# xswang/xflow

Measured on NVIDIA H100. Metric: training examples/sec, higher is better.
Workload: dtype f32

## Files before the change

### xflow_b200/csrc/step_lazy.cu

```cuda
#include <cuda_runtime.h>
#include <stdint.h>
#include <stdlib.h>

#include "kernels.h"
#include "table.cuh"

#define XF_NO_SLOT 0xFFFFFFFFu
#define XF_LAZY_CACHED 2

__global__ void __launch_bounds__(256, 3)
xf_k_step_lr_lazy(XfTableView t, const uint32_t* __restrict__ row_ptr, const uint64_t* __restrict__ keys,
                  const uint8_t* __restrict__ labels, int B, int mode, uint32_t seq, uint32_t* rows_by_seq,
                  float* __restrict__ loss_out, float* __restrict__ pctr_out, float* __restrict__ abs_loss_sum,
                  unsigned long long* __restrict__ unique_total) {
  __shared__ float s_abs[8];
  __shared__ unsigned int s_open;
  if (threadIdx.x == 0) s_open = 0;
  if (blockIdx.x == 0 && threadIdx.x == 0 && mode == 0) rows_by_seq[seq] = (uint32_t)B;
  __syncthreads();
  float abs_acc = 0.f;
  unsigned int open_acc = 0;
  const int lane = threadIdx.x & 31;
  const int warps_per_block = blockDim.x >> 5;
  const int gwarp = blockIdx.x * warps_per_block + (threadIdx.x >> 5);
  const int nwarps = gridDim.x * warps_per_block;

  for (int row = gwarp; row < B; row += nwarps) {
    const uint32_t beg = __ldg(row_ptr + row);
    const uint32_t end = __ldg(row_ptr + row + 1);
    const int chunks = (int)((end - beg + 63u) >> 6);
    float wsum = 0.f;
    uint32_t lead_s[2 * XF_LAZY_CACHED];
    uint32_t cnt_c[XF_LAZY_CACHED];
    uint64_t q2_c[2 * XF_LAZY_CACHED], q3_c[2 * XF_LAZY_CACHED], q2n_c[2 * XF_LAZY_CACHED];
#pragma unroll
    for (int c = 0; c < XF_LAZY_CACHED; ++c) {
      lead_s[2 * c] = lead_s[2 * c + 1] = XF_NO_SLOT;
      q2_c[2 * c] = q2_c[2 * c + 1] = q3_c[2 * c] = q3_c[2 * c + 1] = q2n_c[2 * c] = q2n_c[2 * c + 1] = 0ull;
      cnt_c[c] = 0;
    }

    for (int ch = 0; ch < chunks; ++ch) {
      const uint32_t j0 = beg + (uint32_t)ch * 64u + (uint32_t)lane;
      const uint32_t j1 = j0 + 32u;
      const bool v0 = j0 < end, v1 = j1 < end;
      const uint64_t k0 = v0 ? __ldcs(keys + j0) : 0ull;
      const uint64_t k1 = v1 ? __ldcs(keys + j1) : 0ull;
      const uint64_t p0 = xf_home_slot(t, k0), p1 = xf_home_slot(t, k1);
      XfHead h0, h1;
      h0.key = h1.key = XF_EMPTY_KEY;
      h0.flags = h1.flags = 0u;
      h0.w = h0.n = h0.z = h1.w = h1.n = h1.z = 0.f;
      h0.g = h1.g = 0.0;
      if (v0) h0 = xf_load_head(xf_row(t, p0));
      if (v1) h1 = xf_load_head(xf_row(t, p1));
      uint32_t s0 = XF_NO_SLOT, s1 = XF_NO_SLOT;
      if (v0) { const int64_t r = xf_probe_from<true>(t, k0, p0, h0); if (r >= 0) s0 = (uint32_t)r; }
      if (v1) { const int64_t r = xf_probe_from<true>(t, k1, p1, h1); if (r >= 0) s1 = (uint32_t)r; }
      const uint64_t a2 = xf_raw_q2(h0), a3 = xf_raw_q3(h0), b2 = xf_raw_q2(h1), b3 = xf_raw_q3(h1);
      uint64_t a2n = a2, b2n = b2;
      float w0 = 0.f, w1 = 0.f;
      if (s0 != XF_NO_SLOT) w0 = xf_lazy_fold(t, xf_raw_q1(h0), a2, a3, mode == 1 ? 0xFFFFFFFFu : seq, a2n);
      if (s1 != XF_NO_SLOT) w1 = xf_lazy_fold(t, xf_raw_q1(h1), b2, b3, mode == 1 ? 0xFFFFFFFFu : seq, b2n);
      wsum += w0;
      wsum += w1;
      if (mode == 1) continue;
      const unsigned grp0 = __match_any_sync(0xffffffffu, (s0 != XF_NO_SLOT) ? s0 : (0xFFFFFF00u | (uint32_t)lane));
      const unsigned grp1 = __match_any_sync(0xffffffffu, (s1 != XF_NO_SLOT) ? s1 : (0xFFFFFF00u | (uint32_t)lane));
      const bool L0 = s0 != XF_NO_SLOT && lane == __ffs(grp0) - 1, L1 = s1 != XF_NO_SLOT && lane == __ffs(grp1) - 1;
      if (ch >= XF_LAZY_CACHED) {
        if (L0 && xf_lazy_deposit(t, xf_row(t, s0), a2, a3, a2n, seq, 0ll)) ++open_acc;
        if (L1 && xf_lazy_deposit(t, xf_row(t, s1), b2, b3, b2n, seq, 0ll)) ++open_acc;
      }
#pragma unroll
      for (int c = 0; c < XF_LAZY_CACHED; ++c)
        if (ch == c) {
          lead_s[2 * c] = L0 ? s0 : XF_NO_SLOT;
          lead_s[2 * c + 1] = L1 ? s1 : XF_NO_SLOT;
          q2_c[2 * c] = a2; q3_c[2 * c] = a3; q2n_c[2 * c] = a2n;
          q2_c[2 * c + 1] = b2; q3_c[2 * c + 1] = b3; q2n_c[2 * c + 1] = b2n;
          cnt_c[c] = (L0 ? (uint32_t)__popc(grp0) : 0u) | ((L1 ? (uint32_t)__popc(grp1) : 0u) << 8);
        }
    }

    const float wx = xf_warp_sum(wsum);
    const float pctr = xf_sigmoid(wx);
    if (mode == 1) {
      if (lane == 0 && pctr_out) pctr_out[row] = pctr;
      continue;
    }
    const float loss = __fsub_rn(pctr, (float)labels[row]);
    if (lane == 0 && loss_out) loss_out[row] = loss;
    abs_acc += fabsf(loss);
    const long long lf = xf_fix_of(loss);
#pragma unroll
    for (int c = 0; c < XF_LAZY_CACHED; ++c) {
      if (lead_s[2 * c] != XF_NO_SLOT &&
          xf_lazy_deposit(t, xf_row(t, lead_s[2 * c]), q2_c[2 * c], q3_c[2 * c], q2n_c[2 * c], seq, lf * (long long)(cnt_c[c] & 0xFFu)))
        ++open_acc;
      if (lead_s[2 * c + 1] != XF_NO_SLOT &&
          xf_lazy_deposit(t, xf_row(t, lead_s[2 * c + 1]), q2_c[2 * c + 1], q3_c[2 * c + 1], q2n_c[2 * c + 1], seq,
                          lf * (long long)(cnt_c[c] >> 8)))
        ++open_acc;
    }
    for (int ch = XF_LAZY_CACHED; ch < chunks; ++ch) {
      const uint32_t j0 = beg + (uint32_t)ch * 64u + (uint32_t)lane;
      const uint32_t j1 = j0 + 32u;
      XfHead h;
      if (j0 < end) { const int64_t r = xf_probe<false>(t, __ldg(keys + j0), &h); if (r >= 0) xf_lazy_add(xf_row(t, (uint64_t)r), lf); }
      if (j1 < end) { const int64_t r = xf_probe<false>(t, __ldg(keys + j1), &h); if (r >= 0) xf_lazy_add(xf_row(t, (uint64_t)r), lf); }
    }
  }
  if (mode == 0) {
    if (lane == 0) s_abs[threadIdx.x >> 5] = abs_acc;
    if (open_acc) atomicAdd(&s_open, open_acc);
    __syncthreads();
    if (threadIdx.x == 0) {
      if (abs_loss_sum != nullptr) {
        float tot = 0.f;
        for (int w = 0; w < (int)(blockDim.x >> 5); ++w) tot += s_abs[w];
        atomicAdd(abs_loss_sum, tot);
      }
      if (unique_total != nullptr && s_open) atomicAdd(unique_total, (unsigned long long)s_open);
    }
  }
}

void xf_launch_step_lr_lazy(const XfTableView& t, const uint32_t* row_ptr, const uint64_t* keys,
                            const uint8_t* labels, int B, int mode, uint32_t seq, uint32_t* rows_by_seq,
                            float* loss_out, float* pctr_out, float* abs_loss_sum, unsigned long long* unique_total,
                            cudaStream_t st) {
  if (B <= 0) return;
  const int grid = xf_grid_for((uint64_t)B * 32, 256, 8);
  xf_k_step_lr_lazy<<<grid, 256, 0, st>>>(t, row_ptr, keys, labels, B, mode, seq, rows_by_seq, loss_out, pctr_out,
                                           abs_loss_sum, unique_total);
}
```

### xflow_b200/csrc/table.cuh

```cuda
#pragma once
#include <cuda_runtime.h>
#include <stdint.h>

#define XF_EMPTY_KEY 0xFFFFFFFFFFFFFFFFull
#define XF_FLAG_V_READY 1u
#define XF_NEG_ZERO_BITS 0x80000000u
#define XF_NEG_ZERO_BITS64 0x8000000000000000ull
#define XF_MAX_PROBE 8192

enum { XF_OPT_FTRL = 0, XF_OPT_SGD = 1 };
enum { XF_INIT_DEFAULT = 0, XF_INIT_COUNTER = 1, XF_INIT_ZERO = 3 };

struct XfTableView {
  uint8_t* base;
  uint64_t mask;
  uint32_t log2cap;
  uint32_t bshift;
  uint32_t stride;
  int K;
  int opt;
  int v_init;
  float v_const;
  uint64_t seed;
  float alpha, beta, lambda1, lambda2, learning_rate;
  unsigned long long* size;
  int* error;
  int lazy;
  const uint32_t* rows_by_seq;
  int canon;
};
#define XF_TAG_LOCKED 0xFFFFFFFFu
#define XF_FIX_SCALE 134217728.0
#define XF_FIX_INV 7.450580596923828125e-9
#define XF_TAG_MASK 0xFFFFull

__host__ __device__ inline uint32_t xf_acc_off(int K) { return (32u + 4u * (uint32_t)K + 15u) & ~15u; }
__host__ __device__ inline uint32_t xf_ca_off(int K, int opt) {
  return xf_acc_off(K) + 16u + ((opt == XF_OPT_FTRL) ? 8u * (uint32_t)K : 0u);
}
__host__ __device__ inline uint32_t xf_row_stride(int K, int opt, int canon = 0) {
  if (K <= 0) return 32u;
  uint32_t bytes = xf_ca_off(K, opt) + (canon ? 4u * (uint32_t)K : 0u);
  return (bytes + 31u) & ~31u;
}

#ifdef __CUDACC__

__device__ __forceinline__ uint64_t xf_probe_slot(const XfTableView& t, uint64_t key, uint32_t i) {
  const uint64_t m = key * 0x9E3779B97F4A7C15ull;
  const uint32_t bs = t.bshift;
  const uint64_t hb = m >> (64 - (t.log2cap - bs));
  const uint32_t b1 = (1u << bs) - 1u;
  const uint32_t j0 = (uint32_t)(m >> 9) & b1;
  const uint32_t k = i >> bs;
  const uint32_t j = (k == 0) ? ((j0 + i) & b1) : (i & b1);
  return (((hb + k) << bs) | j) & t.mask;
}
__device__ __forceinline__ uint64_t xf_home_slot(const XfTableView& t, uint64_t key) { return xf_probe_slot(t, key, 0); }

__host__ __device__ __forceinline__ uint64_t xf_splitmix64(uint64_t x) {
  x += 0x9E3779B97F4A7C15ull;
  x = (x ^ (x >> 30)) * 0xBF58476D1CE4E5B9ull;
  x = (x ^ (x >> 27)) * 0x94D049BB133111EBull;
  return x ^ (x >> 31);
}
__device__ __forceinline__ float xf_counter_normal(uint64_t key, uint32_t k, uint64_t seed) {
  uint64_t base = xf_splitmix64(key ^ xf_splitmix64(seed + 0x632BE59BD9B4E019ull * (uint64_t)(k + 1)));
  uint32_t sum = 0;
#pragma unroll
  for (int r = 0; r < 3; ++r) {
    uint64_t x = xf_splitmix64(base + (uint64_t)r);
    sum += (uint32_t)(x & 0xFFFF) + (uint32_t)((x >> 16) & 0xFFFF) + (uint32_t)((x >> 32) & 0xFFFF) +
           (uint32_t)((x >> 48) & 0xFFFF);
  }
  float u = __fmul_rn((float)((int32_t)sum - 6 * 65535), 1.0f / 65536.0f);
  return __fmul_rn(u, 1e-2f);
}
__device__ __forceinline__ float xf_v_init(const XfTableView& t, uint64_t key, uint32_t k) {
  if (t.v_init == XF_INIT_COUNTER) return xf_counter_normal(key, k, t.seed);
  if (t.v_init == XF_INIT_ZERO) return 0.0f;
  return t.v_const;
}

__device__ __forceinline__ uint8_t* xf_row(const XfTableView& t, uint64_t slot) {
  return t.base + slot * (uint64_t)t.stride;
}
__device__ __forceinline__ double* xf_row_g(uint8_t* row) { return reinterpret_cast<double*>(row + 8); }
#define XF_OFF_STATE 16
#define XF_OFF_FLAGS 28
__device__ __forceinline__ float* xf_row_v(uint8_t* row) { return reinterpret_cast<float*>(row + 32); }
__device__ __forceinline__ double* xf_row_acc(uint8_t* row, int K) { return reinterpret_cast<double*>(row + xf_acc_off(K)); }
__device__ __forceinline__ float* xf_row_nv(uint8_t* row, int K) { return reinterpret_cast<float*>(row + xf_acc_off(K) + 16); }
__device__ __forceinline__ float* xf_row_zv(uint8_t* row, int K) { return xf_row_nv(row, K) + K; }
__device__ __forceinline__ float* xf_row_ca(const XfTableView& t, uint8_t* row) { return reinterpret_cast<float*>(row + xf_ca_off(t.K, t.opt)); }

struct XfHead {
  uint64_t key;
  uint32_t flags;
  float w, n, z;
  double g;
};

__device__ __forceinline__ void xf_ld32_cg(const void* p, uint64_t& q0, uint64_t& q1, uint64_t& q2, uint64_t& q3) {
  asm volatile("ld.global.cg.v2.u64 {%0,%1}, [%4];\n\tld.global.cg.v2.u64 {%2,%3}, [%4+16];"
               : "=l"(q0), "=l"(q1), "=l"(q2), "=l"(q3) : "l"(p));
}
__device__ __forceinline__ void xf_ld32_ca(const void* p, uint64_t& q0, uint64_t& q1, uint64_t& q2, uint64_t& q3) {
  asm volatile("ld.global.ca.v2.u64 {%0,%1}, [%4];\n\tld.global.ca.v2.u64 {%2,%3}, [%4+16];"
               : "=l"(q0), "=l"(q1), "=l"(q2), "=l"(q3) : "l"(p));
}
__device__ __forceinline__ void xf_st32(void* p, uint64_t q0, uint64_t q1, uint64_t q2, uint64_t q3) {
  asm volatile("st.global.v2.u64 [%0], {%1,%2};\n\tst.global.v2.u64 [%0+16], {%3,%4};" ::"l"(p), "l"(q0), "l"(q1),
               "l"(q2), "l"(q3)
               : "memory");
}

__device__ __forceinline__ XfHead xf_load_head(const uint8_t* row) {
  uint64_t q0, q1, q2, q3;
  xf_ld32_cg(row, q0, q1, q2, q3);
  XfHead h;
  h.key = q0;
  h.g = __longlong_as_double((long long)q1);
  h.w = __uint_as_float((uint32_t)q2);
  h.n = __uint_as_float((uint32_t)(q2 >> 32));
  h.z = __uint_as_float((uint32_t)q3);
  h.flags = (uint32_t)(q3 >> 32);
  return h;
}

__device__ __forceinline__ XfHead xf_load_head_l1(const uint8_t* row) {
  uint64_t q0, q1, q2, q3;
  xf_ld32_ca(row, q0, q1, q2, q3);
  XfHead h;
  h.key = q0;
  h.g = __longlong_as_double((long long)q1);
  h.w = __uint_as_float((uint32_t)q2);
  h.n = __uint_as_float((uint32_t)(q2 >> 32));
  h.z = __uint_as_float((uint32_t)q3);
  h.flags = (uint32_t)(q3 >> 32);
  return h;
}

__device__ __forceinline__ void xf_ld8_l1(const float* p, float (&o)[8]) {
  uint64_t q0, q1, q2, q3;
  xf_ld32_ca(p, q0, q1, q2, q3);
  o[0] = __uint_as_float((uint32_t)q0); o[1] = __uint_as_float((uint32_t)(q0 >> 32));
  o[2] = __uint_as_float((uint32_t)q1); o[3] = __uint_as_float((uint32_t)(q1 >> 32));
  o[4] = __uint_as_float((uint32_t)q2); o[5] = __uint_as_float((uint32_t)(q2 >> 32));
  o[6] = __uint_as_float((uint32_t)q3); o[7] = __uint_as_float((uint32_t)(q3 >> 32));
}

__device__ __forceinline__ void xf_store_head(uint8_t* row, const XfHead& h) {
  const uint64_t q1 = (uint64_t)__double_as_longlong(h.g);
  const uint64_t q2 = (uint64_t)__float_as_uint(h.w) | ((uint64_t)__float_as_uint(h.n) << 32);
  const uint64_t q3 = (uint64_t)__float_as_uint(h.z) | ((uint64_t)h.flags << 32);
  xf_st32(row, h.key, q1, q2, q3);
}

template <bool INSERT>
__device__ __forceinline__ int64_t xf_probe_from(const XfTableView& t, uint64_t key, uint64_t s, XfHead& h) {
  for (int probes = 0; probes < XF_MAX_PROBE; ++probes) {
    if (h.key == key) return (int64_t)s;
    if (h.key == XF_EMPTY_KEY) {
      if (!INSERT) return -1;
      unsigned long long old =
          atomicCAS(reinterpret_cast<unsigned long long*>(xf_row(t, s)), (unsigned long long)XF_EMPTY_KEY,
                    (unsigned long long)key);
      if (old == XF_EMPTY_KEY) {
        unsigned m = __activemask();
        int leader = __ffs(m) - 1;
        if ((int)(threadIdx.x & 31) == leader) atomicAdd(t.size, (unsigned long long)__popc(m));
        h.key = key; h.flags = 0; h.w = 0.f; h.n = 0.f; h.z = 0.f;
        h.g = t.lazy ? 0.0 : -0.0;
        return (int64_t)s;
      }
      if (old == key) {
        h.key = key;
        return (int64_t)s;
      }
    }
    s = xf_probe_slot(t, key, (uint32_t)probes + 1u);
    h = xf_load_head(xf_row(t, s));
  }
  *t.error = 1;
  return -1;
}

template <bool INSERT>
__device__ __forceinline__ int64_t xf_probe(const XfTableView& t, uint64_t key, XfHead* head) {
  const uint64_t s = xf_home_slot(t, key);
  XfHead h = xf_load_head(xf_row(t, s));
  const int64_t r = xf_probe_from<INSERT>(t, key, s, h);
  *head = h;
  return r;
}


__device__ __forceinline__ float xf_sigmoid(float x) {
  if (x < -30.f) return (float)1e-6;
  if (x > 30.f) return 1.0f;
  const double ex = exp((double)x * 0.9999999998311266);
  return (float)(ex / (1.0 + ex));
}

__device__ __forceinline__ void xf_ftrl_coord(const XfTableView& t, float g, float& w, float& n, float& z) {
  float old_n = n;
  float nn = __fadd_rn(old_n, __fmul_rn(g, g));
  float sig = __fdiv_rn(__fsub_rn(__fsqrt_rn(nn), __fsqrt_rn(old_n)), t.alpha);
  z = __fadd_rn(z, __fsub_rn(g, __fmul_rn(sig, w)));
  n = nn;
  if (fabsf(z) <= t.lambda1) {
    w = 0.0f;
  } else {
    float tmpr = 0.0f;
    if (z > 0.0f) tmpr = __fsub_rn(z, t.lambda1);
    if (z < 0.0f) tmpr = __fadd_rn(z, t.lambda1);
    float tmpl = -__fadd_rn(__fdiv_rn(__fadd_rn(t.beta, __fsqrt_rn(n)), t.alpha), t.lambda2);
    w = __fdiv_rn(tmpr, tmpl);
  }
}

__device__ __forceinline__ void xf_sgd_coord(const XfTableView& t, float g, float& w) {
  w = __fsub_rn(w, __fmul_rn(t.learning_rate, g));
}

__device__ __forceinline__ void xf_opt_coord(const XfTableView& t, float g, float& w, float& n, float& z) {
  if (t.opt == XF_OPT_FTRL) xf_ftrl_coord(t, g, w, n, z);
  else xf_sgd_coord(t, g, w);
}

__device__ __forceinline__ float xf_div_rows_plain(float g, double rows) { return (float)((double)g / rows); }
__device__ __forceinline__ float xf_div_rows(float g, double rows) {
  const long long b = __double_as_longlong(rows);
  if ((b & 0x000FFFFFFFFFFFFFll) == 0ll && b > 0ll) {
    const double inv = __longlong_as_double((2046ll << 52) - b);
    return (float)((double)g * inv);
  }
  return (float)((double)g / rows);
}

__device__ __forceinline__ float xf_ftrl_w(const XfTableView& t, float z, float n) {
  if (fabsf(z) <= t.lambda1) return 0.0f;
  float tmpr = 0.0f;
  if (z > 0.0f) tmpr = __fsub_rn(z, t.lambda1);
  if (z < 0.0f) tmpr = __fadd_rn(z, t.lambda1);
  const float tmpl = -__fadd_rn(__fdiv_rn(__fadd_rn(t.beta, __fsqrt_rn(n)), t.alpha), t.lambda2);
  return __fdiv_rn(tmpr, tmpl);
}
__device__ __forceinline__ long long xf_fix_of(float residual) { return __double2ll_rn((double)residual * XF_FIX_SCALE); }

__device__ __forceinline__ uint64_t xf_raw_q2(const XfHead& h) {
  return (uint64_t)__float_as_uint(h.w) | ((uint64_t)__float_as_uint(h.n) << 32);
}
__device__ __forceinline__ uint64_t xf_raw_q3(const XfHead& h) {
  return (uint64_t)__float_as_uint(h.z) | ((uint64_t)h.flags << 32);
}
__device__ __forceinline__ uint64_t xf_raw_q1(const XfHead& h) { return (uint64_t)__double_as_longlong(h.g); }
__device__ __forceinline__ uint32_t xf_lazy_check(uint64_t q2) {
  const uint32_t c = (uint32_t)q2 ^ (uint32_t)(q2 >> 32) ^ 0xA5A5A5A5u;
  return c ? c : 1u;
}
__device__ __forceinline__ float xf_lazy_fold(const XfTableView& t, uint64_t q1, uint64_t q2, uint64_t q3, uint32_t seq,
                                              uint64_t& q2_new) {
  const uint32_t tag = (uint32_t)(q3 & XF_TAG_MASK);
  const bool pending = tag != 0u && tag != seq;
  float g = 0.f;
  if (pending) {
    const long long gfix = (long long)q3 >> 16;
    g = xf_div_rows_plain((float)((double)gfix * XF_FIX_INV), (double)__ldg(t.rows_by_seq + tag));
  }
  const float a = __uint_as_float((uint32_t)q2), b = __uint_as_float((uint32_t)(q2 >> 32));
  if (t.opt == XF_OPT_FTRL) {
    float n = a, z = b;
    float w = ((uint32_t)(q1 >> 32) == xf_lazy_check(q2)) ? __uint_as_float((uint32_t)q1) : xf_ftrl_w(t, z, n);
    if (pending) xf_ftrl_coord(t, g, w, n, z);
    q2_new = (uint64_t)__float_as_uint(n) | ((uint64_t)__float_as_uint(z) << 32);
    return w;
  }
  float w = a;
  if (pending) xf_sgd_coord(t, g, w);
  q2_new = (uint64_t)__float_as_uint(w);
  return w;
}
__device__ __forceinline__ void xf_apply_pending(const XfTableView& t, XfHead& h) {
  if (!t.lazy) return;
  uint64_t q2n;
  const float w = xf_lazy_fold(t, xf_raw_q1(h), xf_raw_q2(h), xf_raw_q3(h), 0xFFFFFFFFu, q2n);
  h.w = w;
  if (t.opt == XF_OPT_FTRL) {
    h.n = __uint_as_float((uint32_t)q2n);
    h.z = __uint_as_float((uint32_t)(q2n >> 32));
  } else {
    h.n = 0.f;
    h.z = 0.f;
  }
  h.flags = 0u;
  h.g = 0.0;
}
__device__ __forceinline__ bool xf_lazy_has_pending(const XfHead& raw) { return (xf_raw_q3(raw) & XF_TAG_MASK) != 0ull; }
__device__ __forceinline__ void xf_lazy_store(const XfTableView& t, uint8_t* rowp, const XfHead& h, bool keep_w = false) {
  const bool ftrl = t.opt == XF_OPT_FTRL;
  const uint64_t q2 = ftrl ? ((uint64_t)__float_as_uint(h.n) | ((uint64_t)__float_as_uint(h.z) << 32))
                           : (uint64_t)__float_as_uint(h.w);
  uint64_t q1 = 0ull;
  if (keep_w && ftrl && __float_as_uint(h.w) != __float_as_uint(xf_ftrl_w(t, h.z, h.n)))
    q1 = (uint64_t)__float_as_uint(h.w) | ((uint64_t)xf_lazy_check(q2) << 32);
  xf_st32(rowp, h.key, q1, q2, 0ull);
}
__device__ __forceinline__ void xf_store_head_t(const XfTableView& t, uint8_t* rowp, const XfHead& h) {
  if (t.lazy) xf_lazy_store(t, rowp, h);
  else xf_store_head(rowp, h);
}

__device__ __forceinline__ bool xf_cas128(uint8_t* addr, uint64_t e0, uint64_t e1, uint64_t d0, uint64_t d1, uint64_t& o0,
                                          uint64_t& o1) {
  asm volatile(
      "{\n .reg .b128 cmp, swp, old;\n mov.b128 cmp, {%2, %3};\n mov.b128 swp, {%4, %5};\n"
      " atom.global.cas.b128 old, [%6], cmp, swp;\n mov.b128 {%0, %1}, old;\n}"
      : "=l"(o0), "=l"(o1)
      : "l"(e0), "l"(e1), "l"(d0), "l"(d1), "l"(addr)
      : "memory");
  return o0 == e0 && o1 == e1;
}
__device__ __forceinline__ void xf_lazy_add(uint8_t* rowp, long long fix) {
  atomicAdd(reinterpret_cast<unsigned long long*>(rowp + 24), (unsigned long long)fix << 16);
}
__device__ __forceinline__ bool xf_lazy_deposit_issue(uint8_t* rowp, uint64_t q2, uint64_t q3, uint64_t q2_new, uint32_t seq,
                                                      long long fix, uint64_t& o2, uint64_t& o3) {
  if ((uint32_t)(q3 & XF_TAG_MASK) == seq) {
    xf_lazy_add(rowp, fix);
    o2 = q2; o3 = q3;
    return false;
  }
  xf_cas128(rowp + XF_OFF_STATE, q2, q3, q2_new, ((unsigned long long)fix << 16) | (uint64_t)seq, o2, o3);
  return true;
}
__device__ __forceinline__ bool xf_lazy_deposit_resolve(const XfTableView& t, uint8_t* rowp, bool issued, uint64_t q2, uint64_t q3,
                                                        uint64_t o2, uint64_t o3, uint32_t seq, long long fix, bool* stale) {
  if (stale) *stale = false;
  if (!issued) return false;
  if (o2 == q2 && o3 == q3) return true;
  if ((uint32_t)(o3 & XF_TAG_MASK) == seq) {
    xf_lazy_add(rowp, fix);
    return false;
  }
  if (stale) *stale = true;
  else *t.error = 2;
  return false;
}
__device__ __forceinline__ bool xf_lazy_deposit(const XfTableView& t, uint8_t* rowp, uint64_t q2, uint64_t q3, uint64_t q2_new,
                                                uint32_t seq, long long fix, bool* stale = nullptr) {
  if (stale) *stale = false;
  if ((uint32_t)(q3 & XF_TAG_MASK) == seq) {
    xf_lazy_add(rowp, fix);
    return false;
  }
  uint64_t o2, o3;
  if (xf_cas128(rowp + XF_OFF_STATE, q2, q3, q2_new, ((unsigned long long)fix << 16) | (uint64_t)seq, o2, o3)) return true;
  if ((uint32_t)(o3 & XF_TAG_MASK) == seq) {
    xf_lazy_add(rowp, fix);
    return false;
  }
  if (stale) *stale = true;
  else *t.error = 2;
  return false;
}

__device__ __forceinline__ float xf_warp_sum(float v) {
#pragma unroll
  for (int o = 16; o > 0; o >>= 1) v += __shfl_xor_sync(0xffffffffu, v, o);
  return v;
}

#endif
```

Baseline: 77.79 million.

## Pair-share row head loads across lanes and spill cached fold state to shared memory

Replaces the per-lane 32-byte hash-row head load with a cooperative scheme in which adjacent lanes each issue a 16-byte load covering half of both lanes' rows, then exchange halves via shuffles. The probe loop is rewritten inline as a warp-synchronous loop with explicit CAS insertion and batched size counting. The cached per-chunk q2/q3/q2n values for deferred deposits move from registers to shared memory. The goal is fewer wide per-thread loads, better coalescing, and lower register pressure under launch bounds of 3 blocks per SM. The cost is extra shuffles and a larger shared-memory footprint, which may limit occupancy.

New measurement: 83.44 million, median of 6. +7.3%, better.

```diff
diff --git a/xflow_b200/csrc/step_lazy.cu b/xflow_b200/csrc/step_lazy.cu
--- a/xflow_b200/csrc/step_lazy.cu
+++ b/xflow_b200/csrc/step_lazy.cu
@@ -8,6 +8,29 @@
 #define XF_NO_SLOT 0xFFFFFFFFu
 #define XF_LAZY_CACHED 2
 
+__device__ __forceinline__ bool xf_lazy_look(const XfTableView& t, uint64_t key, uint64_t& s, uint32_t& i, uint64_t& q0,
+                                             uint64_t& q1, uint64_t& q2, uint64_t& q3, uint32_t& slot, bool& created) {
+  if (q0 == key) { slot = (uint32_t)s; return true; }
+  if (q0 == XF_EMPTY_KEY) {
+    const unsigned long long old =
+        atomicCAS(reinterpret_cast<unsigned long long*>(xf_row(t, s)), (unsigned long long)XF_EMPTY_KEY, (unsigned long long)key);
+    if (old == XF_EMPTY_KEY) {
+      created = true;
+      q0 = key; q1 = q2 = q3 = 0ull;
+      slot = (uint32_t)s;
+      return true;
+    }
+    if (old == key) {
+      q0 = key;
+      slot = (uint32_t)s;
+      return true;
+    }
+  }
+  if (++i == XF_MAX_PROBE) { *t.error = 1; return true; }
+  s = xf_probe_slot(t, key, i);
+  return false;
+}
+
 __global__ void __launch_bounds__(256, 3)
 xf_k_step_lr_lazy(XfTableView t, const uint32_t* __restrict__ row_ptr, const uint64_t* __restrict__ keys,
                   const uint8_t* __restrict__ labels, int B, int mode, uint32_t seq, uint32_t* rows_by_seq,
@@ -15,6 +38,7 @@
                   unsigned long long* __restrict__ unique_total) {
   __shared__ float s_abs[8];
   __shared__ unsigned int s_open;
+  __shared__ uint64_t s_q2[2 * XF_LAZY_CACHED][256], s_q3[2 * XF_LAZY_CACHED][256], s_q2n[2 * XF_LAZY_CACHED][256];
   if (threadIdx.x == 0) s_open = 0;
   if (blockIdx.x == 0 && threadIdx.x == 0 && mode == 0) rows_by_seq[seq] = (uint32_t)B;
   __syncthreads();
@@ -32,11 +56,9 @@
     float wsum = 0.f;
     uint32_t lead_s[2 * XF_LAZY_CACHED];
     uint32_t cnt_c[XF_LAZY_CACHED];
-    uint64_t q2_c[2 * XF_LAZY_CACHED], q3_c[2 * XF_LAZY_CACHED], q2n_c[2 * XF_LAZY_CACHED];
 #pragma unroll
     for (int c = 0; c < XF_LAZY_CACHED; ++c) {
       lead_s[2 * c] = lead_s[2 * c + 1] = XF_NO_SLOT;
-      q2_c[2 * c] = q2_c[2 * c + 1] = q3_c[2 * c] = q3_c[2 * c + 1] = q2n_c[2 * c] = q2n_c[2 * c + 1] = 0ull;
       cnt_c[c] = 0;
     }
 
@@ -46,22 +68,29 @@
       const bool v0 = j0 < end, v1 = j1 < end;
       const uint64_t k0 = v0 ? __ldcs(keys + j0) : 0ull;
       const uint64_t k1 = v1 ? __ldcs(keys + j1) : 0ull;
-      const uint64_t p0 = xf_home_slot(t, k0), p1 = xf_home_slot(t, k1);
-      XfHead h0, h1;
-      h0.key = h1.key = XF_EMPTY_KEY;
-      h0.flags = h1.flags = 0u;
-      h0.w = h0.n = h0.z = h1.w = h1.n = h1.z = 0.f;
-      h0.g = h1.g = 0.0;
-      if (v0) h0 = xf_load_head(xf_row(t, p0));
-      if (v1) h1 = xf_load_head(xf_row(t, p1));
-      uint32_t s0 = XF_NO_SLOT, s1 = XF_NO_SLOT;
-      if (v0) { const int64_t r = xf_probe_from<true>(t, k0, p0, h0); if (r >= 0) s0 = (uint32_t)r; }
-      if (v1) { const int64_t r = xf_probe_from<true>(t, k1, p1, h1); if (r >= 0) s1 = (uint32_t)r; }
-      const uint64_t a2 = xf_raw_q2(h0), a3 = xf_raw_q3(h0), b2 = xf_raw_q2(h1), b3 = xf_raw_q3(h1);
+      uint64_t p0 = xf_home_slot(t, k0), p1 = xf_home_slot(t, k1);
+      uint64_t a0, a1, a2, a3, b0, b1, b2, b3;
+      xf_ld32_pair(v0 ? xf_row(t, p0) : nullptr, a0, a1, a2, a3);
+      xf_ld32_pair(v1 ? xf_row(t, p1) : nullptr, b0, b1, b2, b3);
+      uint32_t s0 = XF_NO_SLOT, s1 = XF_NO_SLOT, i0 = 0, i1 = 0;
+      bool u0 = v0, u1 = v1;
+      for (;;) {
+        bool c0 = false, c1 = false;
+        if (u0) u0 = !xf_lazy_look(t, k0, p0, i0, a0, a1, a2, a3, s0, c0);
+        if (u1) u1 = !xf_lazy_look(t, k1, p1, i1, b0, b1, b2, b3, s1, c1);
+        const unsigned created = __popc(__ballot_sync(0xffffffffu, c0)) + __popc(__ballot_sync(0xffffffffu, c1));
+        if (created && lane == 0) atomicAdd(t.size, (unsigned long long)created);
+        if (!__any_sync(0xffffffffu, u0 || u1)) break;
+        uint64_t x0, x1, x2, x3;
+        xf_ld32_pair(u0 ? xf_row(t, p0) : nullptr, x0, x1, x2, x3);
+        if (u0) { a0 = x0; a1 = x1; a2 = x2; a3 = x3; }
+        xf_ld32_pair(u1 ? xf_row(t, p1) : nullptr, x0, x1, x2, x3);
+        if (u1) { b0 = x0; b1 = x1; b2 = x2; b3 = x3; }
+      }
       uint64_t a2n = a2, b2n = b2;
       float w0 = 0.f, w1 = 0.f;
-      if (s0 != XF_NO_SLOT) w0 = xf_lazy_fold(t, xf_raw_q1(h0), a2, a3, mode == 1 ? 0xFFFFFFFFu : seq, a2n);
-      if (s1 != XF_NO_SLOT) w1 = xf_lazy_fold(t, xf_raw_q1(h1), b2, b3, mode == 1 ? 0xFFFFFFFFu : seq, b2n);
+      if (s0 != XF_NO_SLOT) w0 = xf_lazy_fold(t, a1, a2, a3, mode == 1 ? 0xFFFFFFFFu : seq, a2n);
+      if (s1 != XF_NO_SLOT) w1 = xf_lazy_fold(t, b1, b2, b3, mode == 1 ? 0xFFFFFFFFu : seq, b2n);
       wsum += w0;
       wsum += w1;
       if (mode == 1) continue;
@@ -77,10 +106,12 @@
         if (ch == c) {
           lead_s[2 * c] = L0 ? s0 : XF_NO_SLOT;
           lead_s[2 * c + 1] = L1 ? s1 : XF_NO_SLOT;
-          q2_c[2 * c] = a2; q3_c[2 * c] = a3; q2n_c[2 * c] = a2n;
-          q2_c[2 * c + 1] = b2; q3_c[2 * c + 1] = b3; q2n_c[2 * c + 1] = b2n;
           cnt_c[c] = (L0 ? (uint32_t)__popc(grp0) : 0u) | ((L1 ? (uint32_t)__popc(grp1) : 0u) << 8);
         }
+      if (ch < XF_LAZY_CACHED) {
+        if (L0) { s_q2[2 * ch][threadIdx.x] = a2; s_q3[2 * ch][threadIdx.x] = a3; s_q2n[2 * ch][threadIdx.x] = a2n; }
+        if (L1) { s_q2[2 * ch + 1][threadIdx.x] = b2; s_q3[2 * ch + 1][threadIdx.x] = b3; s_q2n[2 * ch + 1][threadIdx.x] = b2n; }
+      }
     }
 
     const float wx = xf_warp_sum(wsum);
@@ -95,11 +126,13 @@
     const long long lf = xf_fix_of(loss);
 #pragma unroll
     for (int c = 0; c < XF_LAZY_CACHED; ++c) {
+      const int x = threadIdx.x;
       if (lead_s[2 * c] != XF_NO_SLOT &&
-          xf_lazy_deposit(t, xf_row(t, lead_s[2 * c]), q2_c[2 * c], q3_c[2 * c], q2n_c[2 * c], seq, lf * (long long)(cnt_c[c] & 0xFFu)))
+          xf_lazy_deposit(t, xf_row(t, lead_s[2 * c]), s_q2[2 * c][x], s_q3[2 * c][x], s_q2n[2 * c][x], seq,
+                          lf * (long long)(cnt_c[c] & 0xFFu)))
         ++open_acc;
       if (lead_s[2 * c + 1] != XF_NO_SLOT &&
-          xf_lazy_deposit(t, xf_row(t, lead_s[2 * c + 1]), q2_c[2 * c + 1], q3_c[2 * c + 1], q2n_c[2 * c + 1], seq,
+          xf_lazy_deposit(t, xf_row(t, lead_s[2 * c + 1]), s_q2[2 * c + 1][x], s_q3[2 * c + 1][x], s_q2n[2 * c + 1][x], seq,
                           lf * (long long)(cnt_c[c] >> 8)))
         ++open_acc;
     }
diff --git a/xflow_b200/csrc/table.cuh b/xflow_b200/csrc/table.cuh
--- a/xflow_b200/csrc/table.cuh
+++ b/xflow_b200/csrc/table.cuh
@@ -108,6 +108,22 @@
 __device__ __forceinline__ void xf_ld32_ca(const void* p, uint64_t& q0, uint64_t& q1, uint64_t& q2, uint64_t& q3) {
   asm volatile("ld.global.ca.v2.u64 {%0,%1}, [%4];\n\tld.global.ca.v2.u64 {%2,%3}, [%4+16];"
                : "=l"(q0), "=l"(q1), "=l"(q2), "=l"(q3) : "l"(p));
+}
+__device__ __forceinline__ void xf_ld32_pair(const uint8_t* mine, uint64_t& q0, uint64_t& q1, uint64_t& q2, uint64_t& q3) {
+  const uint32_t odd = threadIdx.x & 1u;
+  const uint8_t* other = (const uint8_t*)__shfl_xor_sync(0xffffffffu, (unsigned long long)mine, 1);
+  const uint8_t* r0 = odd ? other : mine;
+  const uint8_t* r1 = odd ? mine : other;
+  uint64_t x0 = 0, x1 = 0, y0 = 0, y1 = 0;
+  asm volatile("{\n .reg .pred p0, p1;\n setp.ne.u64 p0, %4, 0;\n setp.ne.u64 p1, %5, 0;\n"
+               " @p0 ld.global.cg.v2.u64 {%0,%1}, [%6];\n @p1 ld.global.cg.v2.u64 {%2,%3}, [%7];\n}"
+               : "+l"(x0), "+l"(x1), "+l"(y0), "+l"(y1)
+               : "l"(r0), "l"(r1), "l"(r0 + 16 * odd), "l"(r1 + 16 * odd));
+  const uint64_t m0 = odd ? y0 : x0, m1 = odd ? y1 : x1;
+  const uint64_t t0 = __shfl_xor_sync(0xffffffffu, odd ? x0 : y0, 1);
+  const uint64_t t1 = __shfl_xor_sync(0xffffffffu, odd ? x1 : y1, 1);
+  q0 = odd ? t0 : m0; q1 = odd ? t1 : m1;
+  q2 = odd ? m0 : t0; q3 = odd ? m1 : t1;
 }
 __device__ __forceinline__ void xf_st32(void* p, uint64_t q0, uint64_t q1, uint64_t q2, uint64_t q3) {
   asm volatile("st.global.v2.u64 [%0], {%1,%2};\n\tst.global.v2.u64 [%0+16], {%3,%4};" ::"l"(p), "l"(q0), "l"(q1),
```
